# rakhimovv/lvt

Hardware: AMD Instinct MI355X
Metric: video-clips/sec/node (VQVAE+DSFVT train step, BAIR 64x64x16) (higher is better)
Workload: dtype f32

## Files before the change

### lvt_amd/csrc/epilogue_fast.h

```cpp
#pragma once
#include "lvt_common.h"

typedef float lvt_f32x16 __attribute__((ext_vector_type(16)));

template <int TM, int TN>
__device__ __forceinline__ void lvt_f16x2_finish(lvt_f32x16 (&acc)[TM][TN], lvt_f32x16 (&acx)[TM][TN], int unscale) {
    if (unscale >= -100 && unscale <= 120) {
        const float s = __uint_as_float((unsigned)(unscale + 127) << 23), sx = __uint_as_float((unsigned)(unscale + 116) << 23);
#pragma unroll
        for (int i = 0; i < TM; ++i)
#pragma unroll
            for (int j = 0; j < TN; ++j) acc[i][j] = acx[i][j] * sx + acc[i][j] * s;
    } else {
#pragma unroll
        for (int i = 0; i < TM; ++i)
#pragma unroll
            for (int j = 0; j < TN; ++j)
#pragma unroll
                for (int r = 0; r < 16; ++r) acc[i][j][r] = ldexpf(fmaf(acx[i][j][r], 1.f / 2048.f, acc[i][j][r]), unscale);
    }
}

struct LvtEpi {
    int M, N;
// ... 76 lines not shown
template <int TM, int TN, class RM = LvtRowIdentity>
__device__ __forceinline__ float lvt_epi_fast_dispatch(const LvtEpi &e, lvt_f32x16 (&acc)[TM][TN], float *wave_tile, int m_w, int n_w, int lane,
                                                       const RM rm = RM()) {
#define LVT_EPI_CASE(F) case (F): return lvt_epi_fast_wave<(F), TM, TN, RM>(e, acc, wave_tile, m_w, n_w, lane, rm)
    switch (e.flags & (LVT_EPI_BIAS | LVT_EPI_RESIDUAL | LVT_EPI_RELU | LVT_EPI_MASK)) {
    LVT_EPI_CASE(0);
    LVT_EPI_CASE(LVT_EPI_BIAS);
    LVT_EPI_CASE(LVT_EPI_BIAS | LVT_EPI_RELU);
    LVT_EPI_CASE(LVT_EPI_BIAS | LVT_EPI_RESIDUAL);
    LVT_EPI_CASE(LVT_EPI_BIAS | LVT_EPI_RESIDUAL | LVT_EPI_RELU);
    LVT_EPI_CASE(LVT_EPI_RESIDUAL);
    LVT_EPI_CASE(LVT_EPI_MASK);
    LVT_EPI_CASE(LVT_EPI_RESIDUAL | LVT_EPI_MASK);
    default: return lvt_epi_fast_wave<-1, TM, TN, RM>(e, acc, wave_tile, m_w, n_w, lane, rm);
    }
#undef LVT_EPI_CASE
}

__device__ __forceinline__ unsigned lvt_amax_peek(const float *dst) {
    return (dst && threadIdx.x == 0) ? __hip_atomic_load(reinterpret_cast<const unsigned *>(dst), __ATOMIC_RELAXED, __HIP_MEMORY_SCOPE_AGENT) : 0u;
}
__device__ __forceinline__ void lvt_block_amax_commit_seen(float m, float *dst, float *scratch, unsigned seen) {
#pragma unroll
    for (int d = 32; d > 0; d >>= 1) m = fmaxf(m, __shfl_xor(m, d, 64));
    const int nw = (blockDim.x + 63) >> 6;
    if ((threadIdx.x & 63) == 0) scratch[threadIdx.x >> 6] = m;
    __syncthreads();
    if (threadIdx.x == 0) {
        for (int w = 1; w < nw; ++w) m = fmaxf(m, scratch[w]);
        const unsigned bits = __float_as_uint(m);
        if (bits > seen) atomicMax(reinterpret_cast<unsigned *>(dst), bits);
    }
}
```

### lvt_amd/csrc/gemm_engine.hip

```cpp
#include "lvt_common.h"
#include "epilogue_fast.h"
#include <string.h>
#include <stdlib.h>
#include <stdint.h>
#include <type_traits>

typedef float f32x16 __attribute__((ext_vector_type(16)));

#define BK 32
#define NTHREADS 256

enum { A_KPLAIN = 0, A_MPLAIN = 1, A_CONV_K = 2, A_CONVT_K = 3, A_CONV_M = 4, A_ONEHOT_M = 5, A_PATCH = 6, A_PATCHT = 7 };
enum { B_KPLAIN = 0, B_NPLAIN = 1, B_CONVT_W = 2 };

struct KParams {
    int M, N, K;
    const float *A; long long lda; int a_kb; long long a_skb;
    const float *B; long long ldb; int b_kb; long long b_skb;
    float *C; long long ldc; long long c_plane;
    int batch_inner;
    long long sA_o, sA_i, sB_o, sB_i, sC_o, sC_i;
    float alpha; int flags;
    const float *bias; const float *res; long long ldr; const float *mask; long long ldm;
    int splits; int k_per_split; float *partial; long long partial_stride;
    int vec_epi;
    float *colsum_partial;
    const float *a_amax, *b_amax;
    const float *a_amax2, *b_amax2;
    float *c_amax;
    lvt_conv_geom g;
    const char *b_img;
    int Tq, Hq, Wq;
    int jT, jH, jW;
    const long long *oh_idx; long long oh_bstride, oh_pstride; int oh_P, oh_V; int oh_off[32];
};

__device__ __forceinline__ float4 ldg4(const float *p) { return *reinterpret_cast<const float4 *>(p); }

__device__ __forceinline__ unsigned cvt_pk_bf16(float lo, float hi) {
    unsigned r;
    asm("v_cvt_pk_bf16_f32 %0, %1, %2" : "=v"(r) : "v"(lo), "v"(hi));
    return r;
}
__device__ __forceinline__ float bf_lo(unsigned p) { return __uint_as_float(p << 16); }
__device__ __forceinline__ float bf_hi(unsigned p) { return __uint_as_float(p & 0xffff0000u); }
__device__ __forceinline__ void split3(const float4 v, uint2 &p1, uint2 &p2, uint2 &p3) {
    p1.x = cvt_pk_bf16(v.x, v.y); p1.y = cvt_pk_bf16(v.z, v.w);
    const float r0 = v.x - bf_lo(p1.x), r1 = v.y - bf_hi(p1.x), r2 = v.z - bf_lo(p1.y), r3 = v.w - bf_hi(p1.y);
    p2.x = cvt_pk_bf16(r0, r1); p2.y = cvt_pk_bf16(r2, r3);
    const float s0 = r0 - bf_lo(p2.x), s1 = r1 - bf_hi(p2.x), s2 = r2 - bf_lo(p2.y), s3 = r3 - bf_hi(p2.y);
    p3.x = cvt_pk_bf16(s0, s1); p3.y = cvt_pk_bf16(s2, s3);
}
#define HLD 40
template <int ROWS> __device__ __forceinline__ int hrow(int m) {
    if (ROWS >= 128) {
        const int r = (m & ~127) + ((m & 3) << 5) + ((m & 127) >> 2);
        return r * HLD + (r >> 5) * 32;
    }
    return m * HLD;
}
template <int ROWS> struct HPlane { static constexpr int SIZE = ROWS * HLD + (ROWS >= 128 ? ROWS : 0); };
template <int ROWS> __device__ __forceinline__ void store_split_k(unsigned short *lds, int row, int k4, const float4 v) {
    uint2 p1, p2, p3;
// ... 604 lines not shown
                       (g.sw * qw + rw);
            }
#pragma unroll
            for (int j = 0; j < TN; ++j) {
                const int col = n0 + wn * (TN * 32) + j * 32 + l31;
                if (col >= p.N) continue;
                float v = acc[i][j][r];
                if (p.splits > 1) {
                    p.partial[split * p.partial_stride + (long long)z * p.M * p.N + orow * p.N + col] = v;
                    continue;
                }
                v *= p.alpha;
                if (flags & LVT_EPI_BIAS) v += p.bias[col];
                if (flags & LVT_EPI_RESIDUAL) v += p.res[coff + orow * p.ldr + col];
                if (flags & LVT_EPI_RELU) v = fmaxf(v, 0.f);
                if (flags & LVT_EPI_TANH) v = tanhf(v);
                if (flags & LVT_EPI_SIGMOID) v = lvt_sigmoid_col(v, col < p.N - LVT_EPI_PAD_OF(flags));
                if (flags & LVT_EPI_MASK) v = (p.mask[coff + orow * p.ldm + col] > 0.f) ? v : 0.f;
                float *cp = p.C + coff + orow * p.ldc + col;
                if (flags & LVT_EPI_ACCUM) v += *cp;
                *cp = v;
                am = fmaxf(am, lvt_absf(v));
            }
        }
    }
    if (p.c_amax && p.splits <= 1) {
        __shared__ float amax_scratch[8];
        lvt_block_amax_commit(am, p.c_amax, amax_scratch);
    }
}

struct TileCtx { int m0, n0, z, split, cls, kbeg, kend; const float *A, *B; long long coff; };
template <int AMODE, int BM, int BN>
__device__ __forceinline__ TileCtx lvt_tile_ctx(const KParams &p) {
    TileCtx t;
    const int ntn = (p.N + BN - 1) / BN;
    int wg = blockIdx.x;
    t.split = blockIdx.z;
    t.z = blockIdx.y;
    if (p.splits > 1 && ((gridDim.y * gridDim.z) & 7) == 0) {
        const unsigned lin = blockIdx.x + gridDim.x * (blockIdx.y + gridDim.y * blockIdx.z);
        const unsigned xcd = lin & 7, slot = lin >> 3;
        const unsigned grp = xcd + 8 * (slot / gridDim.x);
        t.z = (int)(grp % gridDim.y);
        t.split = (int)(grp / gridDim.y);
        wg = (int)(slot % gridDim.x);
    } else {
        const int nwg = gridDim.x, q = nwg >> 3, r = nwg & 7;
        const int xcd = wg & 7, slot = wg >> 3;
        wg = (xcd < r ? xcd * (q + 1) : r * (q + 1) + (xcd - r) * q) + slot;
    }
    t.n0 = (wg % ntn) * BN; t.m0 = (wg / ntn) * BM;
    t.A = p.A; t.B = p.B; t.coff = 0; t.cls = 0;
    if (AMODE == A_CONVT_K) {
        t.cls = t.z;
    } else {
        const int zo = t.z / p.batch_inner, zi = t.z % p.batch_inner;
        t.A += zo * p.sA_o + zi * p.sA_i;
        t.B += zo * p.sB_o + zi * p.sB_i;
        t.coff = zo * p.sC_o + zi * p.sC_i;
    }
    t.kbeg = 0; t.kend = p.K;
    if (p.splits > 1) {
        t.kbeg = t.split * p.k_per_split;
        t.kend = min(p.K, t.kbeg + p.k_per_split);
    }
    if (p.flags & LVT_CAUSAL_KMAX) t.kend = min(t.kend, t.m0 + BM);
    if (p.flags & LVT_CAUSAL_KMIN) t.kbeg = max(t.kbeg, (t.m0 / BK) * BK);
    if ((p.flags & LVT_CAUSAL_TILE) && t.n0 > t.m0 + BM - 1) t.kend = t.kbeg;
    return t;
}

template <int AMODE, int BM, int BN, int WM, int WN>
__device__ __forceinline__ void lvt_epilogue_vec(const KParams &p, f32x16 (&acc)[BM / WM / 32][BN / WN / 32], float *lds,
                                                 int m0, int n0, int wm, int wn, int lane, int cls, long long coff, int z,
                                                 int split) {
#pragma clang fp contract(off)
    constexpr int TM = BM / WM / 32, TN = BN / WN / 32;
    constexpr int SW = TN * 32;
    constexpr int C4 = SW / 4;
    const int l31 = lane & 31, half = lane >> 5;
    float *tile = lds + (wm * WN + wn) * (32 * SW);
    int rt = 0, rh = 0, rw = 0;
    if (AMODE == A_CONVT_K) {
        const lvt_conv_geom &g = p.g;
        const int fw = cls % g.sw, fh = (cls / g.sw) % g.sh, ft = cls / (g.sw * g.sh);
        rt = ((ft - g.pt) % g.st + g.st) % g.st;
        rh = ((fh - g.ph) % g.sh + g.sh) % g.sh;
        rw = ((fw - g.pw) % g.sw + g.sw) % g.sw;
    }
    const int flags = p.flags;
    float am = 0.f;
#pragma unroll
    for (int i = 0; i < TM; ++i) {
#pragma unroll
        for (int j = 0; j < TN; ++j)
#pragma unroll
            for (int r = 0; r < 16; ++r) tile[((r & 3) + 8 * (r >> 2) + 4 * half) * SW + 32 * j + l31] = acc[i][j][r];
        __syncthreads();
        if (AMODE != A_KPLAIN && AMODE != A_MPLAIN && p.splits <= 1 && (flags & LVT_EPI_MASK) && !(flags & (LVT_EPI_PLANES | LVT_EPI_ACCUM))) {
            constexpr int NU = 32 * C4 / 64;
            long long oaddr[NU];
            int ocol[NU];
// ... 511 lines not shown
#pragma unroll
                    for (int i = 0; i < TM; ++i)
#pragma unroll
                        for (int j = 0; j < TN; ++j)
                            acc[i][j] = __builtin_amdgcn_mfma_f32_32x32x16_bf16(a[TA[t]][i], b[TB[t]][j], acc[i][j], 0, 0, 0);
            }
        }
        if (!BIMG && has_next && bact) b_store(Bh0 + ((step + 1) & 1) * (NP * PSB));
        if (!DBLA && new_chunk) {
            __syncthreads();
            patch_store(Ah);
        }
        if (BIMG && has_next) b_landed(Bh0 + ((step + 1) & 1) * (NP * PSB));
        __syncthreads();
    }
    if constexpr (MATH == 2) lvt_f16x2_finish<TM, TN>(acc, acx, unscale);
    if (p.vec_epi && p.splits <= 1 && !(p.flags & (LVT_EPI_PLANES | LVT_EPI_ACCUM | LVT_EPI_TANH | LVT_EPI_SIGMOID))) {
        const unsigned seen = lvt_amax_peek(p.c_amax);
        LvtEpi e;
        e.M = p.M; e.N = p.N; e.C = p.C; e.ldc = p.ldc; e.coff = 0; e.alpha = p.alpha; e.flags = p.flags;
        e.bias = p.bias; e.res = p.res; e.ldr = p.ldr; e.mask = p.mask; e.ldm = p.ldm;
        float *wave_tile = lds + wave * (32 * TN * 32);
        float am_w;
        if (MODE != 1) am_w = lvt_epi_fast_dispatch<TM, TN, PatchRows>(e, acc, wave_tile, m0 + wm * (TM * 32), n0 + wn * (TN * 32), lane, PatchRows());
        else am_w = lvt_epi_fast_dispatch<TM, TN, PatchTRows>(e, acc, wave_tile, m0 + wm * (TM * 32), n0 + wn * (TN * 32), lane, PatchTRows{phase});
        if (p.c_amax) lvt_block_amax_commit_seen(am_w, p.c_amax, lds + TURN_FLOATS, seen);
        return;
    }
    if (MODE != 1) lvt_epilogue_vec<A_PATCH, BM, BN, WM, WN>(p, acc, lds, m0, n0, wm, wn, lane, 0, 0, 0, 0);
    else lvt_epilogue_vec<A_PATCHT, BM, BN, WM, WN>(p, acc, lds, m0, n0, wm, wn, lane, phase, 0, 0, 0);
}

#define WIDE_THREADS 512
template <int TA, int TB>
__global__ __launch_bounds__(WIDE_THREADS, 2) void lvt_gemm_wide_kernel(const KParams p) {
    constexpr int BM = 256, BN = 128, WM = 4, WN = 2, TM = 2, TN = 2;
    constexpr int AMODE = TA ? A_MPLAIN : A_KPLAIN;
    constexpr int PSA = HPlane<BM>::SIZE, PSB = HPlane<BN>::SIZE;
    constexpr int STAGE = 2 * (PSA + PSB);
    constexpr int STAGE_FLOATS = (2 * STAGE) / 2 + 8;
    constexpr int TURN_FLOATS = WM * WN * 32 * (TN * 32);
    constexpr int LDS_FLOATS = STAGE_FLOATS > TURN_FLOATS ? STAGE_FLOATS : TURN_FLOATS;
    __shared__ __attribute__((aligned(16))) float lds[LDS_FLOATS];
    unsigned short *S0 = reinterpret_cast<unsigned short *>(lds);

    const int tid = threadIdx.x, lane = tid & 63, wave = tid >> 6;
    const int wm = wave / WN, wn = wave % WN;
    const int l31 = lane & 31, half = lane >> 5;
    const TileCtx tc = lvt_tile_ctx<AMODE, BM, BN>(p);
    const int m0 = tc.m0, n0 = tc.n0, kbeg = tc.kbeg, kend = tc.kend;

    int unscale = 0;
    const float sa = lvt_f16_scale(p.a_amax, unscale, p.a_amax2), sb = lvt_f16_scale(p.b_amax, unscale, p.b_amax2);

    float4 av[4], bv[TB ? 4 : 2];
    const int r0 = tid >> 3, kq = tid & 7;
    const int kk0 = TA ? tid >> 6 : 0, mq = tid & 63;
    const int bkk0 = (tid >> 5) & 7, bnq = tid & 31;
    const bool bact = !TB || tid < 256;
    const char *Ak = reinterpret_cast<const char *>(tc.A), *Bk = reinterpret_cast<const char *>(tc.B);
    unsigned aoff[4], boff_g[TB ? 4 : 2];
    int a_kin = 0, b_kin = 0;
    if (!TA) {
#pragma unroll
        for (int i = 0; i < 4; ++i) aoff[i] = (unsigned)(((long long)min(m0 + r0 + 64 * i, p.M - 1) * p.lda + kq * 4) * 4);
        const int blk = kbeg / p.a_kb;
        a_kin = kbeg - blk * p.a_kb;
        Ak += ((long long)blk * p.a_skb + a_kin) * 4;
    } else {
        const int m = m0 + mq * 4;
#pragma unroll
        for (int i = 0; i < 4; ++i) aoff[i] = (unsigned)(((long long)(kk0 * 4 + i) * p.lda + (m < p.M ? m : 0)) * 4);
        Ak += (long long)kbeg * p.lda * 4;
    }
    if (!TB) {
#pragma unroll
        for (int i = 0; i < 2; ++i) boff_g[i] = (unsigned)(((long long)min(n0 + r0 + 64 * i, p.N - 1) * p.ldb + kq * 4) * 4);
        const int blk = kbeg / p.b_kb;
        b_kin = kbeg - blk * p.b_kb;
        Bk += ((long long)blk * p.b_skb + b_kin) * 4;
    } else {
        const int n = n0 + bnq * 4;
#pragma unroll
        for (int i = 0; i < 4; ++i) boff_g[i] = (unsigned)(((long long)(bkk0 * 4 + i) * p.ldb + (n < p.N ? n : 0)) * 4);
        Bk += (long long)kbeg * p.ldb * 4;
    }
    const bool sum_on = TA && p.colsum_partial != nullptr && n0 == 0;
    float4 colacc = zero4();
    auto fetch = [&]() {
#pragma unroll
        for (int i = 0; i < 4; ++i) av[i] = *reinterpret_cast<const float4 *>(Ak + aoff[i]);
        if (!TA) {
            a_kin += BK;
            const bool wrap = a_kin >= p.a_kb;
            Ak += wrap ? ((long long)p.a_skb - p.a_kb + BK) * 4 : (long long)BK * 4;
            a_kin = wrap ? 0 : a_kin;
        } else {
            Ak += (long long)BK * p.lda * 4;
            if (sum_on) {
#pragma unroll
                for (int i = 0; i < 4; ++i) { colacc.x += av[i].x; colacc.y += av[i].y; colacc.z += av[i].z; colacc.w += av[i].w; }
            }
        }
        if (!TB) {
#pragma unroll
            for (int i = 0; i < 2; ++i) bv[i] = *reinterpret_cast<const float4 *>(Bk + boff_g[i]);
            b_kin += BK;
            const bool wrap = b_kin >= p.b_kb;
            Bk += wrap ? ((long long)p.b_skb - p.b_kb + BK) * 4 : (long long)BK * 4;
            b_kin = wrap ? 0 : b_kin;
        } else {
            if (bact) {
#pragma unroll
                for (int i = 0; i < 4; ++i) bv[i] = *reinterpret_cast<const float4 *>(Bk + boff_g[i]);
            }
            Bk += (long long)BK * p.ldb * 4;
        }
    };
    auto store = [&](unsigned short *buf) {
        unsigned short *Ah = buf, *Bh = buf + 2 * PSA;
        if (!TA) {
#pragma unroll
            for (int i = 0; i < 4; ++i) store_split2_k<BM>(Ah, r0 + 64 * i, kq * 4, av[i], sa);
        } else {
            store_split2_block<BM>(Ah, mq * 4, kk0 * 4, av, sa);
        }
        if (!TB) {
#pragma unroll
            for (int i = 0; i < 2; ++i) store_split2_k<BN>(Bh, r0 + 64 * i, kq * 4, bv[i], sb);
        } else if (bact) {
            store_split2_block<BN>(Bh, bnq * 4, bkk0 * 4, bv, sb);
        }
    };

    f32x16 acc[TM][TN], acx[TM][TN];
#pragma unroll
    for (int i = 0; i < TM; ++i)
#pragma unroll
        for (int j = 0; j < TN; ++j)
#pragma unroll
            for (int r = 0; r < 16; ++r) { acc[i][j][r] = 0.f; acx[i][j][r] = 0.f; }

    int fa[TM], fb[TN];
#pragma unroll
    for (int i = 0; i < TM; ++i) fa[i] = hrow<BM>(wm * (TM * 32) + i * 32 + l31) + 8 * half;
#pragma unroll
    for (int j = 0; j < TN; ++j) fb[j] = 2 * PSA + hrow<BN>(wn * (TN * 32) + j * 32 + l31) + 8 * half;

    auto tile = [&](const unsigned short *cur, unsigned short *nxt, auto do_store, auto do_fetch) {
#pragma unroll
        for (int ks = 0; ks < BK; ks += 16) {
            f16x8 a[2][TM], b[2][TN];
#pragma unroll
            for (int q = 0; q < 2; ++q) {
#pragma unroll
                for (int i = 0; i < TM; ++i) a[q][i] = *reinterpret_cast<const f16x8 *>(cur + fa[i] + q * PSA + ks);
#pragma unroll
                for (int j = 0; j < TN; ++j) b[q][j] = *reinterpret_cast<const f16x8 *>(cur + fb[j] + q * PSB + ks);
            }
#pragma unroll
            for (int i = 0; i < TM; ++i)
#pragma unroll
                for (int j = 0; j < TN; ++j)
                    acx[i][j] = __builtin_amdgcn_mfma_f32_32x32x16_f16(a[0][i], b[1][j], acx[i][j], 0, 0, 0);
#pragma unroll
            for (int i = 0; i < TM; ++i)
#pragma unroll
                for (int j = 0; j < TN; ++j)
                    acc[i][j] = __builtin_amdgcn_mfma_f32_32x32x16_f16(a[0][i], b[0][j], acc[i][j], 0, 0, 0);
#pragma unroll
            for (int i = 0; i < TM; ++i)
#pragma unroll
                for (int j = 0; j < TN; ++j)
                    acx[i][j] = __builtin_amdgcn_mfma_f32_32x32x16_f16(a[1][i], b[0][j], acx[i][j], 0, 0, 0);
            if (ks == 0) {
                if constexpr (decltype(do_store)::value) store(nxt);
                if constexpr (decltype(do_fetch)::value) fetch();
            }
        }
    };
    typedef std::integral_constant<bool, true> yes_t;
    typedef std::integral_constant<bool, false> no_t;

    const int ntiles = kbeg < kend ? (kend - kbeg) / BK : 0;
    if (ntiles > 0) {
        fetch();
        store(S0);
        if (ntiles > 1) fetch();
    }
    __syncthreads();
    int kt = 0;
    for (; kt + 2 < ntiles; ++kt) {
        tile(S0 + (kt & 1) * STAGE, S0 + ((kt + 1) & 1) * STAGE, yes_t(), yes_t());
        __syncthreads();
    }
    if (kt + 1 < ntiles) {
        tile(S0 + (kt & 1) * STAGE, S0 + ((kt + 1) & 1) * STAGE, yes_t(), no_t());
        __syncthreads();
        ++kt;
    }
    if (kt < ntiles) tile(S0 + (kt & 1) * STAGE, nullptr, no_t(), no_t());
    __syncthreads();
    lvt_f16x2_finish<TM, TN>(acc, acx, unscale);

    if (TA && sum_on) {
        float *scratch = lds;
        *reinterpret_cast<float4 *>(&scratch[(kk0 * 64 + mq) * 4]) = colacc;
        __syncthreads();
        if (tid < BM) {
            float s_ = 0.f;
            for (int r = 0; r < 8; ++r) s_ += scratch[(r * 64 + tid / 4) * 4 + (tid & 3)];
            if (m0 + tid < p.M) p.colsum_partial[((long long)tc.split * gridDim.y + tc.z) * p.M + m0 + tid] = s_;
        }
        __syncthreads();
    }
    if (p.vec_epi && !(p.flags & (LVT_EPI_PLANES | LVT_EPI_ACCUM | LVT_EPI_TANH | LVT_EPI_SIGMOID))) {
        LvtEpi e;
        e.M = p.M; e.N = p.N;
        float *wave_tile = lds + wave * (32 * TN * 32);
        if (p.splits > 1) {
            e.C = p.partial; e.ldc = p.N; e.coff = tc.split * p.partial_stride + (long long)tc.z * p.M * p.N; e.alpha = 1.f; e.flags = 0;
            e.bias = nullptr; e.res = nullptr; e.ldr = 0; e.mask = nullptr; e.ldm = 0;
            (void)lvt_epi_fast_wave<0, TM, TN>(e, acc, wave_tile, m0 + wm * (TM * 32), n0 + wn * (TN * 32), lane);
            return;
        }
        const unsigned seen = lvt_amax_peek(p.c_amax);
        e.C = p.C; e.ldc = p.ldc; e.coff = tc.coff; e.alpha = p.alpha; e.flags = p.flags;
        e.bias = p.bias; e.res = p.res; e.ldr = p.ldr; e.mask = p.mask; e.ldm = p.ldm;
        const float am_w = lvt_epi_fast_dispatch<TM, TN>(e, acc, wave_tile, m0 + wm * (TM * 32), n0 + wn * (TN * 32), lane);
        if (p.c_amax) lvt_block_amax_commit_seen(am_w, p.c_amax, lds + TURN_FLOATS, seen);
        return;
    }
    if (p.vec_epi) lvt_epilogue_vec<AMODE, BM, BN, WM, WN>(p, acc, lds, m0, n0, wm, wn, lane, 0, tc.coff, tc.z, tc.split);
    else lvt_epilogue<AMODE, BM, BN, WM, WN>(p, acc, m0, n0, wm, wn, l31, half, 0, tc.coff, tc.z, tc.split);
}

__global__ void lvt_reduce_splits_kernel(const float *__restrict__ partial, long long n4, long long stride,
                                         int splits, float *__restrict__ out, int accumulate) {
    long long i = (long long)blockIdx.x * blockDim.x + threadIdx.x;
    const long long step = (long long)gridDim.x * blockDim.x;
    for (; i < n4; i += step) {
        float4 s0 = ldg4(partial + i * 4), s1 = zero4(), s2 = zero4(), s3 = zero4();
        int k = 1;
        for (; k + 3 < splits; k += 4) {
            const float4 t0 = ldg4(partial + k * stride + i * 4), t1 = ldg4(partial + (k + 1) * stride + i * 4);
            const float4 t2 = ldg4(partial + (k + 2) * stride + i * 4), t3 = ldg4(partial + (k + 3) * stride + i * 4);
            s0.x += t0.x; s0.y += t0.y; s0.z += t0.z; s0.w += t0.w;
            s1.x += t1.x; s1.y += t1.y; s1.z += t1.z; s1.w += t1.w;
            s2.x += t2.x; s2.y += t2.y; s2.z += t2.z; s2.w += t2.w;
            s3.x += t3.x; s3.y += t3.y; s3.z += t3.z; s3.w += t3.w;
        }
        for (; k < splits; ++k) {
            const float4 t = ldg4(partial + k * stride + i * 4);
            s0.x += t.x; s0.y += t.y; s0.z += t.z; s0.w += t.w;
        }
        float4 s;
        s.x = (s0.x + s1.x) + (s2.x + s3.x); s.y = (s0.y + s1.y) + (s2.y + s3.y);
        s.z = (s0.z + s1.z) + (s2.z + s3.z); s.w = (s0.w + s1.w) + (s2.w + s3.w);
        float4 *o = reinterpret_cast<float4 *>(out + i * 4);
        if (accumulate) { const float4 c = *o; s.x += c.x; s.y += c.y; s.z += c.z; s.w += c.w; }
        *o = s;
    }
}

__global__ void lvt_pack_weight_kernel(const float *__restrict__ w, float *__restrict__ wp, int taps, int Ci,
                                       int Co, int Ci_real, int Co_real) {
    const long long total = (long long)taps * Ci * Co;
// ... 149 lines not shown
    const long long ntm = lvt_cdiv(p.M, BM), ntn = lvt_cdiv(p.N, BN);
    if (ntm * ntn > 0x7fffffffLL || zcount > 65535 || p.splits > 65535) {
        lvt_set_error("gemm: grid too large (%lld tiles, z=%d, splits=%d)", ntm * ntn, zcount, p.splits);
        return LVT_EINVAL;
    }
    dim3 grid((unsigned)(ntm * ntn), (unsigned)zcount, (unsigned)(p.splits > 1 ? p.splits : 1));
    KParams pv = p;
    {
        auto al16 = [](const void *q) { return ((uintptr_t)q & 15) == 0; };
        bool ok = p.N % 4 == 0;
        if (p.splits > 1) ok = ok && al16(p.partial) && p.partial_stride % 4 == 0 && ((long long)p.M * p.N) % 4 == 0;
        else {
            ok = ok && al16(p.C) && p.ldc % 4 == 0 && p.sC_o % 4 == 0 && p.sC_i % 4 == 0;
            if (p.flags & LVT_EPI_BIAS) ok = ok && al16(p.bias);
            if (p.flags & LVT_EPI_RESIDUAL) ok = ok && al16(p.res) && p.ldr % 4 == 0;
            if (p.flags & LVT_EPI_MASK) ok = ok && al16(p.mask) && p.ldm % 4 == 0;
        }
        pv.vec_epi = ok ? 1 : 0;
    }
    if ((p.flags & LVT_EPI_PLANES) && !pv.vec_epi) {
        lvt_set_error("gemm: LVT_EPI_PLANES needs 16-byte aligned bias / res / mask and ldr, ldm %% 4 == 0");
        return LVT_EINVAL;
    }
    if (math_of(p.flags) == 2)
        hipLaunchKernelGGL((lvt_gemm_kernel<AMODE, BMODE, BM, BN, WM, WN, 2>), grid, dim3(NTHREADS), 0, s, pv);
    else if (math_of(p.flags) == 1)
        hipLaunchKernelGGL((lvt_gemm_kernel<AMODE, BMODE, BM, BN, WM, WN, 1>), grid, dim3(NTHREADS), 0, s, pv);
    else
        hipLaunchKernelGGL((lvt_gemm_kernel<AMODE, BMODE, BM, BN, WM, WN, 0>), grid, dim3(NTHREADS), 0, s, pv);
    LVT_CHECK_LAUNCH("lvt_gemm_kernel");
    return LVT_OK;
}

template <int TA, int TB>
static int launch_wide(const KParams &p, int zcount, hipStream_t s) {
    const long long ntm = lvt_cdiv(p.M, 256), ntn = lvt_cdiv(p.N, 128);
    if (ntm * ntn > 0x7fffffffLL || zcount > 65535 || p.splits > 65535) {
        lvt_set_error("gemm: grid too large (%lld tiles, z=%d, splits=%d)", ntm * ntn, zcount, p.splits);
        return LVT_EINVAL;
    }
    dim3 grid((unsigned)(ntm * ntn), (unsigned)zcount, (unsigned)(p.splits > 1 ? p.splits : 1));
    KParams pv = p;
    {
        auto al16 = [](const void *q) { return ((uintptr_t)q & 15) == 0; };
        bool ok = p.N % 4 == 0;
        if (p.splits > 1) ok = ok && al16(p.partial) && p.partial_stride % 4 == 0 && ((long long)p.M * p.N) % 4 == 0;
        else {
            ok = ok && al16(p.C) && p.ldc % 4 == 0 && p.sC_o % 4 == 0 && p.sC_i % 4 == 0;
            if (p.flags & LVT_EPI_BIAS) ok = ok && al16(p.bias);
            if (p.flags & LVT_EPI_RESIDUAL) ok = ok && al16(p.res) && p.ldr % 4 == 0;
            if (p.flags & LVT_EPI_MASK) ok = ok && al16(p.mask) && p.ldm % 4 == 0;
        }
        pv.vec_epi = ok ? 1 : 0;
    }
    if ((p.flags & LVT_EPI_PLANES) && !pv.vec_epi) {
        lvt_set_error("gemm: LVT_EPI_PLANES needs 16-byte aligned bias / res / mask and ldr, ldm %% 4 == 0");
        return LVT_EINVAL;
    }
    hipLaunchKernelGGL((lvt_gemm_wide_kernel<TA, TB>), grid, dim3(WIDE_THREADS), 0, s, pv);
    LVT_CHECK_LAUNCH("lvt_gemm_wide_kernel");
    return LVT_OK;
}

static int choose_splits(long long tiles, int K, int min_k) {
    int s = (int)((2 * LVT_NUM_CU) / (tiles > 0 ? tiles : 1));
    const int maxs = K / min_k > 0 ? K / min_k : 1;
    if (s > maxs) s = maxs;
    if (s < 1) s = 1;
    return s;
}

static void kparams_from_desc(const lvt_gemm_desc *d, KParams &p) {
    memset(&p, 0, sizeof(p));
    p.M = d->M; p.N = d->N; p.K = d->K;
    p.A = d->A; p.lda = d->lda; p.a_kb = d->a_kb > 0 ? d->a_kb : d->K; p.a_skb = d->a_skb;
// ... 616 lines not shown
```

Baseline: 1336.

## Make wide GEMM kernel persistent with next-tile prefetch overlapping epilogue

For the TB==0 wide GEMM, the grid is capped at the number of CUs (rounded to a multiple of 8), and each workgroup loops over virtual tiles. The next tile's setup and first global fetch are issued before the current tile's epilogue, so load latency overlaps with output stores. The amax reduction is accumulated per wave across tiles and committed once per block, and kernel params are reloaded from the kernarg segment to limit register pressure. This removes wave-launch tail overhead and repeated prologue latency, but one block per CU may cut occupancy relative to launch_bounds of 2, and it adds loop complexity.

```diff
diff --git a/lvt_amd/csrc/epilogue_fast.h b/lvt_amd/csrc/epilogue_fast.h
--- a/lvt_amd/csrc/epilogue_fast.h
+++ b/lvt_amd/csrc/epilogue_fast.h
@@ -132,3 +132,21 @@
         if (bits > seen) atomicMax(reinterpret_cast<unsigned *>(dst), bits);
     }
 }
+
+__device__ __forceinline__ unsigned lvt_wave_amax_bits(float m) {
+#pragma unroll
+    for (int d = 32; d > 0; d >>= 1) m = fmaxf(m, __shfl_xor(m, d, 64));
+    return __builtin_amdgcn_readfirstlane(__float_as_uint(m));
+}
+__device__ __forceinline__ void lvt_block_amax_commit_waves(unsigned wave_bits, float *dst, unsigned *scratch, unsigned seen) {
+    const int nw = (blockDim.x + 63) >> 6;
+    int tid = threadIdx.x;
+    asm volatile("" : "+v"(tid));
+    if ((tid & 63) == 0) scratch[tid >> 6] = wave_bits;
+    __syncthreads();
+    if (tid == 0) {
+        unsigned bits = wave_bits;
+        for (int w = 1; w < nw; ++w) bits = max(bits, scratch[w]);
+        if (bits > seen) atomicMax(reinterpret_cast<unsigned *>(dst), bits);
+    }
+}
diff --git a/lvt_amd/csrc/gemm_engine.hip b/lvt_amd/csrc/gemm_engine.hip
--- a/lvt_amd/csrc/gemm_engine.hip
+++ b/lvt_amd/csrc/gemm_engine.hip
@@ -4,6 +4,7 @@
 #include <stdlib.h>
 #include <stdint.h>
 #include <type_traits>
+#include <atomic>
 
 typedef float f32x16 __attribute__((ext_vector_type(16)));
 
@@ -29,6 +30,7 @@
     const float *a_amax2, *b_amax2;
     float *c_amax;
     lvt_conv_geom g;
+    unsigned vgx, vgy, vgz;
     const char *b_img;
     int Tq, Hq, Wq;
     int jT, jH, jW;
@@ -699,21 +701,22 @@
 
 struct TileCtx { int m0, n0, z, split, cls, kbeg, kend; const float *A, *B; long long coff; };
 template <int AMODE, int BM, int BN>
-__device__ __forceinline__ TileCtx lvt_tile_ctx(const KParams &p) {
+__device__ __forceinline__ TileCtx lvt_tile_ctx(const KParams &p, unsigned bx, unsigned by, unsigned bz, unsigned gx, unsigned gy,
+                                                unsigned gz) {
     TileCtx t;
     const int ntn = (p.N + BN - 1) / BN;
-    int wg = blockIdx.x;
-    t.split = blockIdx.z;
-    t.z = blockIdx.y;
-    if (p.splits > 1 && ((gridDim.y * gridDim.z) & 7) == 0) {
-        const unsigned lin = blockIdx.x + gridDim.x * (blockIdx.y + gridDim.y * blockIdx.z);
+    int wg = bx;
+    t.split = bz;
+    t.z = by;
+    if (p.splits > 1 && ((gy * gz) & 7) == 0) {
+        const unsigned lin = bx + gx * (by + gy * bz);
         const unsigned xcd = lin & 7, slot = lin >> 3;
-        const unsigned grp = xcd + 8 * (slot / gridDim.x);
-        t.z = (int)(grp % gridDim.y);
-        t.split = (int)(grp / gridDim.y);
-        wg = (int)(slot % gridDim.x);
+        const unsigned grp = xcd + 8 * (slot / gx);
+        t.z = (int)(grp % gy);
+        t.split = (int)(grp / gy);
+        wg = (int)(slot % gx);
     } else {
-        const int nwg = gridDim.x, q = nwg >> 3, r = nwg & 7;
+        const int nwg = gx, q = nwg >> 3, r = nwg & 7;
         const int xcd = wg & 7, slot = wg >> 3;
         wg = (xcd < r ? xcd * (q + 1) : r * (q + 1) + (xcd - r) * q) + slot;
     }
@@ -736,6 +739,10 @@
     if (p.flags & LVT_CAUSAL_KMIN) t.kbeg = max(t.kbeg, (t.m0 / BK) * BK);
     if ((p.flags & LVT_CAUSAL_TILE) && t.n0 > t.m0 + BM - 1) t.kend = t.kbeg;
     return t;
+}
+template <int AMODE, int BM, int BN>
+__device__ __forceinline__ TileCtx lvt_tile_ctx(const KParams &p) {
+    return lvt_tile_ctx<AMODE, BM, BN>(p, blockIdx.x, blockIdx.y, blockIdx.z, gridDim.x, gridDim.y, gridDim.z);
 }
 
 template <int AMODE, int BM, int BN, int WM, int WN>
@@ -1313,10 +1320,18 @@
 }
 
 #define WIDE_THREADS 512
+typedef const __attribute__((address_space(4))) KParams *lvt_kparams_karg;
+__device__ __forceinline__ void lvt_kparams_reload(KParams &dst) {
+    lvt_kparams_karg q = (lvt_kparams_karg)__builtin_amdgcn_kernarg_segment_ptr();
+    asm volatile("" : "+s"(q));
+    __builtin_memcpy(&dst, q, sizeof(KParams));
+}
+template <int TA, int TB> struct WideLoop { static constexpr bool value = TB == 0; };
 template <int TA, int TB>
 __global__ __launch_bounds__(WIDE_THREADS, 2) void lvt_gemm_wide_kernel(const KParams p) {
     constexpr int BM = 256, BN = 128, WM = 4, WN = 2, TM = 2, TN = 2;
     constexpr int AMODE = TA ? A_MPLAIN : A_KPLAIN;
+    constexpr bool LOOP = WideLoop<TA, TB>::value;
     constexpr int PSA = HPlane<BM>::SIZE, PSB = HPlane<BN>::SIZE;
     constexpr int STAGE = 2 * (PSA + PSB);
     constexpr int STAGE_FLOATS = (2 * STAGE) / 2 + 8;
@@ -1325,59 +1340,79 @@
     __shared__ __attribute__((aligned(16))) float lds[LDS_FLOATS];
     unsigned short *S0 = reinterpret_cast<unsigned short *>(lds);
 
-    const int tid = threadIdx.x, lane = tid & 63, wave = tid >> 6;
-    const int wm = wave / WN, wn = wave % WN;
-    const int l31 = lane & 31, half = lane >> 5;
-    const TileCtx tc = lvt_tile_ctx<AMODE, BM, BN>(p);
-    const int m0 = tc.m0, n0 = tc.n0, kbeg = tc.kbeg, kend = tc.kend;
-
-    int unscale = 0;
-    const float sa = lvt_f16_scale(p.a_amax, unscale, p.a_amax2), sb = lvt_f16_scale(p.b_amax, unscale, p.b_amax2);
+    const int tid = threadIdx.x;
+    const unsigned G = gridDim.x * gridDim.y * gridDim.z, vtotal = p.vgx * p.vgy * p.vgz;
+    unsigned v = blockIdx.x + gridDim.x * (blockIdx.y + gridDim.y * blockIdx.z);
+
+    int unscale_v = 0;
+    const float sa_v = lvt_f16_scale(p.a_amax, unscale_v, p.a_amax2), sb_v = lvt_f16_scale(p.b_amax, unscale_v, p.b_amax2);
+    const float sa = __uint_as_float(__builtin_amdgcn_readfirstlane(__float_as_uint(sa_v)));
+    const float sb = __uint_as_float(__builtin_amdgcn_readfirstlane(__float_as_uint(sb_v)));
+    const int unscale = __builtin_amdgcn_readfirstlane(unscale_v);
 
     float4 av[4], bv[TB ? 4 : 2];
-    const int r0 = tid >> 3, kq = tid & 7;
-    const int kk0 = TA ? tid >> 6 : 0, mq = tid & 63;
-    const int bkk0 = (tid >> 5) & 7, bnq = tid & 31;
-    const bool bact = !TB || tid < 256;
-    const char *Ak = reinterpret_cast<const char *>(tc.A), *Bk = reinterpret_cast<const char *>(tc.B);
+    int r0, kq;
+    int kk0, mq;
+    int bkk0, bnq;
+    bool bact;
+    KParams pk;
+    const char *Ak, *Bk;
     unsigned aoff[4], boff_g[TB ? 4 : 2];
     int a_kin = 0, b_kin = 0;
-    if (!TA) {
-#pragma unroll
-        for (int i = 0; i < 4; ++i) aoff[i] = (unsigned)(((long long)min(m0 + r0 + 64 * i, p.M - 1) * p.lda + kq * 4) * 4);
-        const int blk = kbeg / p.a_kb;
-        a_kin = kbeg - blk * p.a_kb;
-        Ak += ((long long)blk * p.a_skb + a_kin) * 4;
-    } else {
-        const int m = m0 + mq * 4;
-#pragma unroll
-        for (int i = 0; i < 4; ++i) aoff[i] = (unsigned)(((long long)(kk0 * 4 + i) * p.lda + (m < p.M ? m : 0)) * 4);
-        Ak += (long long)kbeg * p.lda * 4;
-    }
-    if (!TB) {
-#pragma unroll
-        for (int i = 0; i < 2; ++i) boff_g[i] = (unsigned)(((long long)min(n0 + r0 + 64 * i, p.N - 1) * p.ldb + kq * 4) * 4);
-        const int blk = kbeg / p.b_kb;
-        b_kin = kbeg - blk * p.b_kb;
-        Bk += ((long long)blk * p.b_skb + b_kin) * 4;
-    } else {
-        const int n = n0 + bnq * 4;
-#pragma unroll
-        for (int i = 0; i < 4; ++i) boff_g[i] = (unsigned)(((long long)(bkk0 * 4 + i) * p.ldb + (n < p.N ? n : 0)) * 4);
-        Bk += (long long)kbeg * p.ldb * 4;
-    }
-    const bool sum_on = TA && p.colsum_partial != nullptr && n0 == 0;
+    bool sum_on = false;
     float4 colacc = zero4();
+    int ntiles = 0;
+    auto setup = [&](unsigned vt) {
+        lvt_kparams_reload(pk);
+        const KParams &p = pk;
+        const unsigned vrow = vt / p.vgx;
+        const TileCtx tc = lvt_tile_ctx<AMODE, BM, BN>(p, vt - vrow * p.vgx, vrow % p.vgy, vrow / p.vgy, p.vgx, p.vgy, p.vgz);
+        const int m0 = tc.m0, n0 = tc.n0, kbeg = tc.kbeg;
+        int tid_s = tid;
+        asm volatile("" : "+v"(tid_s));
+        bact = !TB || tid_s < 256;
+        const int r0 = tid_s >> 3, kq = tid_s & 7, kk0 = TA ? tid_s >> 6 : 0, mq = tid_s & 63, bkk0 = (tid_s >> 5) & 7, bnq = tid_s & 31;
+        Ak = reinterpret_cast<const char *>(tc.A); Bk = reinterpret_cast<const char *>(tc.B);
+        a_kin = 0; b_kin = 0;
+        if (!TA) {
+#pragma unroll
+            for (int i = 0; i < 4; ++i) aoff[i] = (unsigned)(((long long)min(m0 + r0 + 64 * i, p.M - 1) * p.lda + kq * 4) * 4);
+            const int blk = kbeg / p.a_kb;
+            a_kin = kbeg - blk * p.a_kb;
+            Ak += ((long long)blk * p.a_skb + a_kin) * 4;
+        } else {
+            const int m = m0 + mq * 4;
+#pragma unroll
+            for (int i = 0; i < 4; ++i) aoff[i] = (unsigned)(((long long)(kk0 * 4 + i) * p.lda + (m < p.M ? m : 0)) * 4);
+            Ak += (long long)kbeg * p.lda * 4;
+        }
+        if (!TB) {
+#pragma unroll
+            for (int i = 0; i < 2; ++i) boff_g[i] = (unsigned)(((long long)min(n0 + r0 + 64 * i, p.N - 1) * p.ldb + kq * 4) * 4);
+            const int blk = kbeg / p.b_kb;
+            b_kin = kbeg - blk * p.b_kb;
+            Bk += ((long long)blk * p.b_skb + b_kin) * 4;
+        } else {
+            const int n = n0 + bnq * 4;
+#pragma unroll
+            for (int i = 0; i < 4; ++i) boff_g[i] = (unsigned)(((long long)(bkk0 * 4 + i) * p.ldb + (n < p.N ? n : 0)) * 4);
+            Bk += (long long)kbeg * p.ldb * 4;
+        }
+        sum_on = TA && p.colsum_partial != nullptr && n0 == 0;
+        colacc = zero4();
+        ntiles = kbeg < tc.kend ? (tc.kend - kbeg) / BK : 0;
+        return tc;
+    };
     auto fetch = [&]() {
 #pragma unroll
         for (int i = 0; i < 4; ++i) av[i] = *reinterpret_cast<const float4 *>(Ak + aoff[i]);
         if (!TA) {
             a_kin += BK;
-            const bool wrap = a_kin >= p.a_kb;
-            Ak += wrap ? ((long long)p.a_skb - p.a_kb + BK) * 4 : (long long)BK * 4;
+            const bool wrap = a_kin >= pk.a_kb;
+            Ak += wrap ? ((long long)pk.a_skb - pk.a_kb + BK) * 4 : (long long)BK * 4;
             a_kin = wrap ? 0 : a_kin;
         } else {
-            Ak += (long long)BK * p.lda * 4;
+            Ak += (long long)BK * pk.lda * 4;
             if (sum_on) {
 #pragma unroll
                 for (int i = 0; i < 4; ++i) { colacc.x += av[i].x; colacc.y += av[i].y; colacc.z += av[i].z; colacc.w += av[i].w; }
@@ -1387,15 +1422,15 @@
 #pragma unroll
             for (int i = 0; i < 2; ++i) bv[i] = *reinterpret_cast<const float4 *>(Bk + boff_g[i]);
             b_kin += BK;
-            const bool wrap = b_kin >= p.b_kb;
-            Bk += wrap ? ((long long)p.b_skb - p.b_kb + BK) * 4 : (long long)BK * 4;
+            const bool wrap = b_kin >= pk.b_kb;
+            Bk += wrap ? ((long long)pk.b_skb - pk.b_kb + BK) * 4 : (long long)BK * 4;
             b_kin = wrap ? 0 : b_kin;
         } else {
             if (bact) {
 #pragma unroll
                 for (int i = 0; i < 4; ++i) bv[i] = *reinterpret_cast<const float4 *>(Bk + boff_g[i]);
             }
-            Bk += (long long)BK * p.ldb * 4;
+            Bk += (long long)BK * pk.ldb * 4;
         }
     };
     auto store = [&](unsigned short *buf) {
@@ -1415,18 +1450,7 @@
     };
 
     f32x16 acc[TM][TN], acx[TM][TN];
-#pragma unroll
-    for (int i = 0; i < TM; ++i)
-#pragma unroll
-        for (int j = 0; j < TN; ++j)
-#pragma unroll
-            for (int r = 0; r < 16; ++r) { acc[i][j][r] = 0.f; acx[i][j][r] = 0.f; }
-
     int fa[TM], fb[TN];
-#pragma unroll
-    for (int i = 0; i < TM; ++i) fa[i] = hrow<BM>(wm * (TM * 32) + i * 32 + l31) + 8 * half;
-#pragma unroll
-    for (int j = 0; j < TN; ++j) fb[j] = 2 * PSA + hrow<BN>(wn * (TN * 32) + j * 32 + l31) + 8 * half;
 
     auto tile = [&](const unsigned short *cur, unsigned short *nxt, auto do_store, auto do_fetch) {
 #pragma unroll
@@ -1463,57 +1487,101 @@
     typedef std::integral_constant<bool, true> yes_t;
     typedef std::integral_constant<bool, false> no_t;
 
-    const int ntiles = kbeg < kend ? (kend - kbeg) / BK : 0;
-    if (ntiles > 0) {
-        fetch();
-        store(S0);
-        if (ntiles > 1) fetch();
-    }
-    __syncthreads();
-    int kt = 0;
-    for (; kt + 2 < ntiles; ++kt) {
-        tile(S0 + (kt & 1) * STAGE, S0 + ((kt + 1) & 1) * STAGE, yes_t(), yes_t());
+    unsigned am_run = 0;
+    unsigned seen = 0;
+
+    TileCtx tc = setup(v);
+    if (ntiles > 0) fetch();
+    for (;;) {
+        {
+            int tid_f = tid;
+            asm volatile("" : "+v"(tid_f));
+            const int wave_f = tid_f >> 6, l31_f = tid_f & 31, half_f = (tid_f >> 5) & 1;
+            r0 = tid_f >> 3; kq = tid_f & 7; kk0 = TA ? tid_f >> 6 : 0; mq = tid_f & 63; bkk0 = (tid_f >> 5) & 7; bnq = tid_f & 31;
+            bact = !TB || tid_f < 256;
+#pragma unroll
+            for (int i = 0; i < TM; ++i) fa[i] = hrow<BM>((wave_f / WN) * (TM * 32) + i * 32 + l31_f) + 8 * half_f;
+#pragma unroll
+            for (int j = 0; j < TN; ++j) fb[j] = 2 * PSA + hrow<BN>((wave_f % WN) * (TN * 32) + j * 32 + l31_f) + 8 * half_f;
+        }
+#pragma unroll
+        for (int i = 0; i < TM; ++i)
+#pragma unroll
+            for (int j = 0; j < TN; ++j)
+#pragma unroll
+                for (int r = 0; r < 16; ++r) { acc[i][j][r] = 0.f; acx[i][j][r] = 0.f; }
+        if (ntiles > 0) {
+            store(S0);
+            if (ntiles > 1) fetch();
+        }
         __syncthreads();
-    }
-    if (kt + 1 < ntiles) {
-        tile(S0 + (kt & 1) * STAGE, S0 + ((kt + 1) & 1) * STAGE, yes_t(), no_t());
+        int kt = 0;
+        for (; kt + 2 < ntiles; ++kt) {
+            tile(S0 + (kt & 1) * STAGE, S0 + ((kt + 1) & 1) * STAGE, yes_t(), yes_t());
+            __syncthreads();
+        }
+        if (kt + 1 < ntiles) {
+            tile(S0 + (kt & 1) * STAGE, S0 + ((kt + 1) & 1) * STAGE, yes_t(), no_t());
+            __syncthreads();
+            ++kt;
+        }
+        if (kt < ntiles) tile(S0 + (kt & 1) * STAGE, nullptr, no_t(), no_t());
         __syncthreads();
-        ++kt;
-    }
-    if (kt < ntiles) tile(S0 + (kt & 1) * STAGE, nullptr, no_t(), no_t());
-    __syncthreads();
-    lvt_f16x2_finish<TM, TN>(acc, acx, unscale);
-
-    if (TA && sum_on) {
-        float *scratch = lds;
-        *reinterpret_cast<float4 *>(&scratch[(kk0 * 64 + mq) * 4]) = colacc;
+        lvt_f16x2_finish<TM, TN>(acc, acx, unscale);
+
+        KParams pe;
+        lvt_kparams_reload(pe);
+        const int m0 = tc.m0, n0 = tc.n0;
+        if (TA && sum_on) {
+            float *scratch = lds;
+            *reinterpret_cast<float4 *>(&scratch[(kk0 * 64 + mq) * 4]) = colacc;
+            __syncthreads();
+            if (tid < BM) {
+                float s_ = 0.f;
+                for (int r = 0; r < 8; ++r) s_ += scratch[(r * 64 + tid / 4) * 4 + (tid & 3)];
+                if (m0 + tid < pe.M) pe.colsum_partial[((long long)tc.split * pe.vgy + tc.z) * pe.M + m0 + tid] = s_;
+            }
+            __syncthreads();
+        }
+        const unsigned vn = v + G;
+        const bool more = LOOP && vn < vtotal && vn > v;
+        int tid_e = tid;
+        asm volatile("" : "+v"(tid_e));
+        const int lane_e = tid_e & 63, wave_e = tid_e >> 6, wm_e = wave_e / WN, wn_e = wave_e % WN;
+        float *wave_tile = lds + wave_e * (32 * TN * 32);
+        const TileCtx te = tc;
+        if (pe.vec_epi && !(pe.flags & (LVT_EPI_PLANES | LVT_EPI_ACCUM | LVT_EPI_TANH | LVT_EPI_SIGMOID))) {
+            if (more) {
+                tc = setup(vn);
+                if (ntiles > 0) fetch();
+            }
+            LvtEpi e;
+            e.M = pe.M; e.N = pe.N;
+            if (pe.splits > 1) {
+                e.C = pe.partial; e.ldc = pe.N; e.coff = te.split * pe.partial_stride + (long long)te.z * pe.M * pe.N; e.alpha = 1.f; e.flags = 0;
+                e.bias = nullptr; e.res = nullptr; e.ldr = 0; e.mask = nullptr; e.ldm = 0;
+                (void)lvt_epi_fast_wave<0, TM, TN>(e, acc, wave_tile, m0 + wm_e * (TM * 32), n0 + wn_e * (TN * 32), lane_e);
+            } else {
+                if (!more) seen = lvt_amax_peek(pe.c_amax);
+                e.C = pe.C; e.ldc = pe.ldc; e.coff = te.coff; e.alpha = pe.alpha; e.flags = pe.flags;
+                e.bias = pe.bias; e.res = pe.res; e.ldr = pe.ldr; e.mask = pe.mask; e.ldm = pe.ldm;
+                const float am_w = lvt_epi_fast_dispatch<TM, TN>(e, acc, wave_tile, m0 + wm_e * (TM * 32), n0 + wn_e * (TN * 32), lane_e);
+                am_run = max(am_run, lvt_wave_amax_bits(am_w));
+            }
+        } else {
+            if (pe.vec_epi) lvt_epilogue_vec<AMODE, BM, BN, WM, WN>(pe, acc, lds, m0, n0, wm_e, wn_e, lane_e, 0, te.coff, te.z, te.split);
+            else lvt_epilogue<AMODE, BM, BN, WM, WN>(pe, acc, m0, n0, wm_e, wn_e, lane_e & 31, lane_e >> 5, 0, te.coff, te.z, te.split);
+            if (more) {
+                tc = setup(vn);
+                if (ntiles > 0) fetch();
+            }
+        }
+        if (!more) break;
+        v = vn;
         __syncthreads();
-        if (tid < BM) {
-            float s_ = 0.f;
-            for (int r = 0; r < 8; ++r) s_ += scratch[(r * 64 + tid / 4) * 4 + (tid & 3)];
-            if (m0 + tid < p.M) p.colsum_partial[((long long)tc.split * gridDim.y + tc.z) * p.M + m0 + tid] = s_;
-        }
-        __syncthreads();
-    }
-    if (p.vec_epi && !(p.flags & (LVT_EPI_PLANES | LVT_EPI_ACCUM | LVT_EPI_TANH | LVT_EPI_SIGMOID))) {
-        LvtEpi e;
-        e.M = p.M; e.N = p.N;
-        float *wave_tile = lds + wave * (32 * TN * 32);
-        if (p.splits > 1) {
-            e.C = p.partial; e.ldc = p.N; e.coff = tc.split * p.partial_stride + (long long)tc.z * p.M * p.N; e.alpha = 1.f; e.flags = 0;
-            e.bias = nullptr; e.res = nullptr; e.ldr = 0; e.mask = nullptr; e.ldm = 0;
-            (void)lvt_epi_fast_wave<0, TM, TN>(e, acc, wave_tile, m0 + wm * (TM * 32), n0 + wn * (TN * 32), lane);
-            return;
-        }
-        const unsigned seen = lvt_amax_peek(p.c_amax);
-        e.C = p.C; e.ldc = p.ldc; e.coff = tc.coff; e.alpha = p.alpha; e.flags = p.flags;
-        e.bias = p.bias; e.res = p.res; e.ldr = p.ldr; e.mask = p.mask; e.ldm = p.ldm;
-        const float am_w = lvt_epi_fast_dispatch<TM, TN>(e, acc, wave_tile, m0 + wm * (TM * 32), n0 + wn * (TN * 32), lane);
-        if (p.c_amax) lvt_block_amax_commit_seen(am_w, p.c_amax, lds + TURN_FLOATS, seen);
-        return;
-    }
-    if (p.vec_epi) lvt_epilogue_vec<AMODE, BM, BN, WM, WN>(p, acc, lds, m0, n0, wm, wn, lane, 0, tc.coff, tc.z, tc.split);
-    else lvt_epilogue<AMODE, BM, BN, WM, WN>(p, acc, m0, n0, wm, wn, l31, half, 0, tc.coff, tc.z, tc.split);
+    }
+    if (p.c_amax && p.splits <= 1 && p.vec_epi && !(p.flags & (LVT_EPI_PLANES | LVT_EPI_ACCUM | LVT_EPI_TANH | LVT_EPI_SIGMOID)))
+        lvt_block_amax_commit_waves(am_run, p.c_amax, reinterpret_cast<unsigned *>(lds + TURN_FLOATS), seen);
 }
 
 __global__ void lvt_reduce_splits_kernel(const float *__restrict__ partial, long long n4, long long stride,
@@ -1729,6 +1797,20 @@
     return LVT_OK;
 }
 
+static int wide_resident_workgroups() {
+    static std::atomic<int> cached[64];
+    int dev = 0;
+    if (hipGetDevice(&dev) != hipSuccess || dev < 0 || dev >= 64) return LVT_NUM_CU & ~7;
+    int r = cached[dev].load(std::memory_order_relaxed);
+    if (r == 0) {
+        int cus = 0;
+        if (hipDeviceGetAttribute(&cus, hipDeviceAttributeMultiprocessorCount, dev) != hipSuccess || cus < 8) cus = LVT_NUM_CU;
+        r = cus & ~7;
+        cached[dev].store(r, std::memory_order_relaxed);
+    }
+    return r;
+}
+
 template <int TA, int TB>
 static int launch_wide(const KParams &p, int zcount, hipStream_t s) {
     const long long ntm = lvt_cdiv(p.M, 256), ntn = lvt_cdiv(p.N, 128);
@@ -1736,8 +1818,17 @@
         lvt_set_error("gemm: grid too large (%lld tiles, z=%d, splits=%d)", ntm * ntn, zcount, p.splits);
         return LVT_EINVAL;
     }
-    dim3 grid((unsigned)(ntm * ntn), (unsigned)zcount, (unsigned)(p.splits > 1 ? p.splits : 1));
+    const unsigned nsplit = (unsigned)(p.splits > 1 ? p.splits : 1);
+    const long long total = ntm * ntn * zcount * nsplit;
+    if (total > 0x7fffffffLL) {
+        lvt_set_error("gemm: grid too large (%lld tiles, z=%d, splits=%d)", ntm * ntn, zcount, p.splits);
+        return LVT_EINVAL;
+    }
+    const int R = wide_resident_workgroups();
+    dim3 grid((unsigned)(ntm * ntn), (unsigned)zcount, nsplit);
+    if (WideLoop<TA, TB>::value && total > R) grid = dim3((unsigned)R, 1, 1);
     KParams pv = p;
+    pv.vgx = (unsigned)(ntm * ntn); pv.vgy = (unsigned)zcount; pv.vgz = nsplit;
     {
         auto al16 = [](const void *q) { return ((uintptr_t)q & 15) == 0; };
         bool ok = p.N % 4 == 0;
```

After: 1331. About the same (-0.4%).

## Store transposed wide-GEMM operands in memory order and read with ds_read_tr16

Applied to the files above, without the earlier changes.

For transposed A/B operands in the wide GEMM kernel, the LDS image is now kept in K-major memory order with a padded pitch, and MFMA fragments are assembled with the gfx950 transposing LDS read (ds_read_tr16_b64). This replaces the transpose-on-store path with simple 8-byte stores. The B loader is also rebalanced so all 512 threads each load two float4 instead of half the threads loading four. The intent is to cut LDS store cost and bank conflicts in the transposed layouts, at the cost of relying on the transposing-read lane mapping being correct.

```diff
diff --git a/lvt_amd/csrc/gemm_engine.hip b/lvt_amd/csrc/gemm_engine.hip
--- a/lvt_amd/csrc/gemm_engine.hip
+++ b/lvt_amd/csrc/gemm_engine.hip
@@ -1313,12 +1313,26 @@
 }
 
 #define WIDE_THREADS 512
+#define WT_PA (256 + 32)
+#define WT_PB (128 + 32)
+typedef short s16x4 __attribute__((ext_vector_type(4)));
+__device__ __forceinline__ f16x8 wide_tr_frag(const unsigned short *p, int pitch4) {
+    typedef __attribute__((address_space(3))) s16x4 lds_v4;
+    const s16x4 lo = __builtin_amdgcn_ds_read_tr16_b64_v4i16((lds_v4 *)(p));
+    const s16x4 hi = __builtin_amdgcn_ds_read_tr16_b64_v4i16((lds_v4 *)(p + pitch4));
+    union { struct { s16x4 a, b; } s; f16x8 v; } u;
+    u.s.a = lo; u.s.b = hi;
+    return u.v;
+}
 template <int TA, int TB>
 __global__ __launch_bounds__(WIDE_THREADS, 2) void lvt_gemm_wide_kernel(const KParams p) {
     constexpr int BM = 256, BN = 128, WM = 4, WN = 2, TM = 2, TN = 2;
     constexpr int AMODE = TA ? A_MPLAIN : A_KPLAIN;
-    constexpr int PSA = HPlane<BM>::SIZE, PSB = HPlane<BN>::SIZE;
+    constexpr int PA = WT_PA, PB = WT_PB;
+    constexpr int PSA = TA ? BK * PA : HPlane<BM>::SIZE, PSB = TB ? BK * PB : HPlane<BN>::SIZE;
     constexpr int STAGE = 2 * (PSA + PSB);
+    static_assert(PA % 4 == 0 && PB % 4 == 0 && PSA % 8 == 0 && PSB % 8 == 0, "transposing reads need 8-byte aligned addresses");
+    static_assert(BK * PA <= HPlane<BM>::SIZE && BK * PB <= HPlane<BN>::SIZE, "the memory-order images are the smaller ones");
     constexpr int STAGE_FLOATS = (2 * STAGE) / 2 + 8;
     constexpr int TURN_FLOATS = WM * WN * 32 * (TN * 32);
     constexpr int LDS_FLOATS = STAGE_FLOATS > TURN_FLOATS ? STAGE_FLOATS : TURN_FLOATS;
@@ -1334,13 +1348,12 @@
     int unscale = 0;
     const float sa = lvt_f16_scale(p.a_amax, unscale, p.a_amax2), sb = lvt_f16_scale(p.b_amax, unscale, p.b_amax2);
 
-    float4 av[4], bv[TB ? 4 : 2];
+    float4 av[4], bv[2];
     const int r0 = tid >> 3, kq = tid & 7;
     const int kk0 = TA ? tid >> 6 : 0, mq = tid & 63;
-    const int bkk0 = (tid >> 5) & 7, bnq = tid & 31;
-    const bool bact = !TB || tid < 256;
+    const int bkk0 = tid >> 5, bnq = tid & 31;
     const char *Ak = reinterpret_cast<const char *>(tc.A), *Bk = reinterpret_cast<const char *>(tc.B);
-    unsigned aoff[4], boff_g[TB ? 4 : 2];
+    unsigned aoff[4], boff_g[2];
     int a_kin = 0, b_kin = 0;
     if (!TA) {
 #pragma unroll
@@ -1363,7 +1376,7 @@
     } else {
         const int n = n0 + bnq * 4;
 #pragma unroll
-        for (int i = 0; i < 4; ++i) boff_g[i] = (unsigned)(((long long)(bkk0 * 4 + i) * p.ldb + (n < p.N ? n : 0)) * 4);
+        for (int i = 0; i < 2; ++i) boff_g[i] = (unsigned)(((long long)(bkk0 * 2 + i) * p.ldb + (n < p.N ? n : 0)) * 4);
         Bk += (long long)kbeg * p.ldb * 4;
     }
     const bool sum_on = TA && p.colsum_partial != nullptr && n0 == 0;
@@ -1391,10 +1404,8 @@
             Bk += wrap ? ((long long)p.b_skb - p.b_kb + BK) * 4 : (long long)BK * 4;
             b_kin = wrap ? 0 : b_kin;
         } else {
-            if (bact) {
-#pragma unroll
-                for (int i = 0; i < 4; ++i) bv[i] = *reinterpret_cast<const float4 *>(Bk + boff_g[i]);
-            }
+#pragma unroll
+            for (int i = 0; i < 2; ++i) bv[i] = *reinterpret_cast<const float4 *>(Bk + boff_g[i]);
             Bk += (long long)BK * p.ldb * 4;
         }
     };
@@ -1404,13 +1415,27 @@
 #pragma unroll
             for (int i = 0; i < 4; ++i) store_split2_k<BM>(Ah, r0 + 64 * i, kq * 4, av[i], sa);
         } else {
-            store_split2_block<BM>(Ah, mq * 4, kk0 * 4, av, sa);
+#pragma unroll
+            for (int i = 0; i < 4; ++i) {
+                uint2 ph, pl;
+                split2(av[i], sa, ph, pl);
+                unsigned short *d = Ah + (kk0 * 4 + i) * PA + mq * 4;
+                *reinterpret_cast<uint2 *>(d) = ph;
+                *reinterpret_cast<uint2 *>(d + PSA) = pl;
+            }
         }
         if (!TB) {
 #pragma unroll
             for (int i = 0; i < 2; ++i) store_split2_k<BN>(Bh, r0 + 64 * i, kq * 4, bv[i], sb);
-        } else if (bact) {
-            store_split2_block<BN>(Bh, bnq * 4, bkk0 * 4, bv, sb);
+        } else {
+#pragma unroll
+            for (int i = 0; i < 2; ++i) {
+                uint2 ph, pl;
+                split2(bv[i], sb, ph, pl);
+                unsigned short *d = Bh + (bkk0 * 2 + i) * PB + bnq * 4;
+                *reinterpret_cast<uint2 *>(d) = ph;
+                *reinterpret_cast<uint2 *>(d + PSB) = pl;
+            }
         }
     };
 
@@ -1422,11 +1447,13 @@
 #pragma unroll
             for (int r = 0; r < 16; ++r) { acc[i][j][r] = 0.f; acx[i][j][r] = 0.f; }
 
+    const int trow = 8 * half + ((lane & 15) >> 2), tcol = (lane & 16) + 4 * (lane & 3);
     int fa[TM], fb[TN];
 #pragma unroll
-    for (int i = 0; i < TM; ++i) fa[i] = hrow<BM>(wm * (TM * 32) + i * 32 + l31) + 8 * half;
-#pragma unroll
-    for (int j = 0; j < TN; ++j) fb[j] = 2 * PSA + hrow<BN>(wn * (TN * 32) + j * 32 + l31) + 8 * half;
+    for (int i = 0; i < TM; ++i) fa[i] = TA ? trow * PA + wm * (TM * 32) + i * 32 + tcol : hrow<BM>(wm * (TM * 32) + i * 32 + l31) + 8 * half;
+#pragma unroll
+    for (int j = 0; j < TN; ++j)
+        fb[j] = 2 * PSA + (TB ? trow * PB + wn * (TN * 32) + j * 32 + tcol : hrow<BN>(wn * (TN * 32) + j * 32 + l31) + 8 * half);
 
     auto tile = [&](const unsigned short *cur, unsigned short *nxt, auto do_store, auto do_fetch) {
 #pragma unroll
@@ -1435,9 +1462,15 @@
 #pragma unroll
             for (int q = 0; q < 2; ++q) {
 #pragma unroll
-                for (int i = 0; i < TM; ++i) a[q][i] = *reinterpret_cast<const f16x8 *>(cur + fa[i] + q * PSA + ks);
-#pragma unroll
-                for (int j = 0; j < TN; ++j) b[q][j] = *reinterpret_cast<const f16x8 *>(cur + fb[j] + q * PSB + ks);
+                for (int i = 0; i < TM; ++i) {
+                    if constexpr (TA) a[q][i] = wide_tr_frag(cur + fa[i] + q * PSA + ks * PA, 4 * PA);
+                    else a[q][i] = *reinterpret_cast<const f16x8 *>(cur + fa[i] + q * PSA + ks);
+                }
+#pragma unroll
+                for (int j = 0; j < TN; ++j) {
+                    if constexpr (TB) b[q][j] = wide_tr_frag(cur + fb[j] + q * PSB + ks * PB, 4 * PB);
+                    else b[q][j] = *reinterpret_cast<const f16x8 *>(cur + fb[j] + q * PSB + ks);
+                }
             }
 #pragma unroll
             for (int i = 0; i < TM; ++i)
```

New measurement: 1417 before, 1432 after (median of 6 runs). 1.01x the previous value.
